# facebook/zstd

Measured on NVIDIA H100. Metric: compress GB/s (input) at level 1, higher is better.
Workload: dtype u8

## Files before the change

### zstd_b200/csrc/zb_api.cu

```cuda
#include <cuda_runtime.h>
#include <stdio.h>
#include <stdlib.h>
#include <string.h>
#include <vector>
#include <mutex>
#include <thread>
#include <new>
#include <time.h>
#include "../../include/zstd_b200.h"
#include "zb_common.h"
#include "zb_kernels.h"

static inline u32 hb32(u32 v) { return 31u - (u32)__builtin_clz(v); }

typedef struct { u32 windowLog, chainLog, hashLog, searchLog, minMatch, targetLength, strategy; } ZbCParams;
struct Row { u8 W, C, H, S, L, TL, strat; };
static const Row kRows[4][5] = {
    { {19,12,13,1,6,1,1}, {19,13,14,1,7,0,1}, {20,15,16,1,6,0,1}, {21,16,17,1,5,0,2}, {21,18,18,1,5,0,2} },
    { {18,12,13,1,5,1,1}, {18,13,14,1,6,0,1}, {18,14,14,1,5,0,2}, {18,16,16,1,4,0,2}, {18,16,16,1,4,0,2} },
    { {17,12,12,1,5,1,1}, {17,12,13,1,6,0,1}, {17,13,15,1,5,0,1}, {17,15,16,2,5,0,2}, {17,17,17,2,4,0,2} },
    { {14,12,13,1,5,1,1}, {14,14,15,1,5,0,1}, {14,14,15,1,4,0,1}, {14,14,15,2,4,0,2}, {14,14,15,2,4,0,2} },
};

static ZbCParams zb_getCParams(int level, u64 srcSize, size_t dictSize)
// ... 55 lines not shown
#define ZB_IMAGE_BYTES (ZB_IMAGE_WORDS * 4u)
#define ZB_MAX_IMAGES 4

#include <atomic>
static std::atomic<int> g_device(-1);

#define ZB_WAVE_SLOTS_MAX 14u
#define ZB_WAVE_SLOTS_DEFAULT 4u
#define ZB_HOST_WAVE_SLOTS_DEFAULT 8u
#define ZB_HOST_WAVE_BLOCKS 384u
struct ZSTD_CDict_s {
    int level;
    const u8* content;
    size_t size;
    size_t contentOff, tail;
    ZbDictEntropy entropy;
    std::mutex* lock;
    int device;
    bool resident;
    u8* d_dict; ZbDictEntropy* d_de; u8* d_image; ZbChunk* d_dictChunk;
    u32 nbImages; ZbParams imagePrm[ZB_MAX_IMAGES];
};

struct ZbPlan;
static void zb_freePlan(struct ZbPlan* p);
struct ZSTD_CCtx_s {
    int device;
    int bindDevice;
    cudaStream_t stream;
    size_t capBlocks, capFrames, capWaves;
    size_t capHeavyBytes[9];
    size_t capChunks; ZbChunk* d_chunks;
    ZbSegMeta* d_segmeta;
    u32 devWaveBlocks;
    cudaStream_t waveStream[ZB_WAVE_SLOTS_MAX + 1];
    u32 waveSlots;
    u32 hostWaveSlots;
    u32 hostWaveBlocks;
    ZbBlock* d_blocks; ZbFrame* d_frames; ZbBlockMeta* d_meta;
    u64* d_seqs; u8* d_lits; u8* d_body; u16* d_dist;
    u16* d_dist2;
    u32* d_far; u32* d_far2;
    u64* d_outOffsets; u64* d_frameSizes; u64* d_totals;
    u8* d_in; size_t d_inCap; u8* d_out; size_t d_outCap;
    ZSTD_CDict* callDict;
    u64* h_totals;
    cudaEvent_t evStart, evK0, evMid, evK1, evK2, evK3, evKEnd, evEnd;
    cudaEvent_t* evWave;
    u32 capEvWaves; bool evWaveTimed;
    ZSTDB200_stats stats;
    int advLevel, advChecksum, advNoDictID;
    ZSTD_CDict* advLocalDict;
    const ZSTD_CDict* advRefCDict;
    struct ZbPlan* plan;
    u8* stIn; size_t stInSize, stInCap;
    u8* stOut; size_t stOutSize, stOutPos, stOutCap;
    int stFrames;
    int advDelims;
    u8* d_seqIn; size_t d_seqInCap;
    void* d_seqTile; size_t d_seqTileCap; void* d_seqBlk; size_t d_seqBlkCap; u64* d_seqCtrl;
};

static double zb_now(void) { struct timespec ts; clock_gettime(CLOCK_MONOTONIC, &ts); return (double)ts.tv_sec + 1e-9 * (double)ts.tv_nsec; }

extern "C" int ZSTDB200_setDevice(int device) { g_device.store(device); return 0; }
int zb_contextDevice(void)
// ... 32 lines not shown
static size_t zb_ctxInit(ZSTD_CCtx* c)
{
    if (c->device >= 0) { CK(cudaSetDevice(c->device)); return 0; }
    int n = 0;
    if (cudaGetDeviceCount(&n) != cudaSuccess || n == 0) { cudaGetLastError(); return ZB_ERR(ZB_error_GENERIC); }
    int dev = c->bindDevice;
    if (dev < 0) { if (cudaGetDevice(&dev) != cudaSuccess) dev = 0; }
    CK(cudaSetDevice(dev));
    cudaStream_t st = nullptr; cudaEvent_t ev[8] = { nullptr, nullptr, nullptr, nullptr, nullptr, nullptr, nullptr, nullptr };
    cudaError_t e = cudaStreamCreateWithFlags(&st, cudaStreamNonBlocking);
    for (int i = 0; i < 8 && e == cudaSuccess; i++) e = cudaEventCreate(&ev[i]);
    if (e == cudaSuccess) {
        static ZbdFseCTable defaults[3]; static std::once_flag once;
        std::call_once(once, [] { zb_buildDefaultTables(defaults); });
        e = zb_upload_default_tables(defaults, st);
        if (e == cudaSuccess) e = cudaStreamSynchronize(st);
    }
    if (e != cudaSuccess) {
        for (int i = 0; i < 8; i++) if (ev[i]) cudaEventDestroy(ev[i]);
        if (st) cudaStreamDestroy(st);
        cudaGetLastError();
        return ZB_ERR(e == cudaErrorMemoryAllocation ? ZB_error_memory_allocation : ZB_error_GENERIC);
    }
    c->stream = st;
    c->evStart = ev[0]; c->evK0 = ev[1]; c->evK1 = ev[2]; c->evK2 = ev[3]; c->evK3 = ev[4]; c->evMid = ev[5]; c->evKEnd = ev[6]; c->evEnd = ev[7];
    c->device = dev;
    return 0;
}

static void zb_freeWorkspace(ZSTD_CCtx* c)
{
    cudaFree(c->d_blocks); cudaFree(c->d_frames); cudaFree(c->d_meta); cudaFree(c->d_seqs); cudaFree(c->d_lits);
    cudaFree(c->d_body); cudaFree(c->d_dist); cudaFree(c->d_dist2); c->d_dist2 = NULL; cudaFree(c->d_segmeta); c->d_segmeta = NULL;
    cudaFree(c->d_far); cudaFree(c->d_far2); c->d_far = NULL; c->d_far2 = NULL; cudaFree(c->d_chunks); c->d_chunks = NULL; c->capChunks = 0; cudaFree(c->d_outOffsets); cudaFree(c->d_frameSizes); cudaFree(c->d_totals);
    cudaFreeHost(c->h_totals);
    c->d_blocks = NULL; c->d_frames = NULL; c->d_meta = NULL; c->d_seqs = NULL; c->d_lits = NULL;
    c->d_body = NULL; c->d_dist = NULL; c->d_outOffsets = NULL; c->d_frameSizes = NULL; c->d_totals = NULL; c->h_totals = NULL;
    c->capBlocks = 0; c->capFrames = 0; c->capWaves = 0; memset(c->capHeavyBytes, 0, sizeof(c->capHeavyBytes));
}

static void zb_freeWaveEvents(ZSTD_CCtx* c)
{
    for (u32 i = 0; i < 4u * c->capEvWaves; i++) if (c->evWave[i]) cudaEventDestroy(c->evWave[i]);
    free(c->evWave); c->evWave = NULL; c->capEvWaves = 0;
}
static size_t zb_ensureWaveEvents(ZSTD_CCtx* c, u32 nbWaves, bool timed)
{
    if (nbWaves <= c->capEvWaves && timed == c->evWaveTimed) return 0;
    zb_freeWaveEvents(c);
    c->evWave = (cudaEvent_t*)calloc(4u * nbWaves, sizeof(cudaEvent_t));
    if (!c->evWave) return ZB_ERR(ZB_error_memory_allocation);
    c->capEvWaves = nbWaves; c->evWaveTimed = timed;
    for (u32 i = 0; i < 4u * nbWaves; i++) {
        cudaError_t const e = cudaEventCreateWithFlags(&c->evWave[i], timed ? cudaEventDefault : cudaEventDisableTiming);
        if (e != cudaSuccess) { zb_freeWaveEvents(c); CK(e); }
    }
    return 0;
}

extern "C" size_t ZSTD_freeCDict(ZSTD_CDict* cd);
extern "C" size_t ZSTD_freeCCtx(ZSTD_CCtx* c)
{
    if (!c) return 0;
    ZbDeviceGuard guard;
    ZSTD_freeCDict(c->advLocalDict); ZSTD_freeCDict(c->callDict);
    free(c->stIn); free(c->stOut);
    zb_freePlan(c->plan);
    if (c->device >= 0) {
        cudaSetDevice(c->device);
        zb_freeWorkspace(c);
        zb_freeWaveEvents(c);
        cudaFree(c->d_in); cudaFree(c->d_out);
        cudaFree(c->d_seqIn); cudaFree(c->d_seqTile); cudaFree(c->d_seqBlk); cudaFree(c->d_seqCtrl);
        for (u32 s = 0; s <= ZB_WAVE_SLOTS_MAX; s++) if (c->waveStream[s]) cudaStreamDestroy(c->waveStream[s]);
        cudaEventDestroy(c->evStart); cudaEventDestroy(c->evK0); cudaEventDestroy(c->evK1);
        cudaEventDestroy(c->evK2); cudaEventDestroy(c->evK3); cudaEventDestroy(c->evMid);
        cudaEventDestroy(c->evKEnd); cudaEventDestroy(c->evEnd);
        cudaStreamDestroy(c->stream);
    }
    free(c);
    return 0;
}

static size_t zb_ensureDesc(ZSTD_CCtx* c, size_t nbBlocks, size_t nbFrames, size_t nbWaves, size_t nbChunks)
{
    if (nbChunks > c->capChunks) {
        cudaFree(c->d_chunks); c->d_chunks = NULL; c->capChunks = 0;
        CK(cudaMalloc(&c->d_chunks, nbChunks * sizeof(ZbChunk)));
        c->capChunks = nbChunks;
    }
    if (nbBlocks > c->capBlocks) {
        cudaFree(c->d_blocks); cudaFree(c->d_outOffsets); c->d_blocks = NULL; c->d_outOffsets = NULL; c->capBlocks = 0;
        CK(cudaMalloc(&c->d_blocks, nbBlocks * sizeof(ZbBlock)));
        CK(cudaMalloc(&c->d_outOffsets, (nbBlocks + 1) * sizeof(u64)));
        c->capBlocks = nbBlocks;
    }
    if (nbFrames > c->capFrames) {
        cudaFree(c->d_frames); cudaFree(c->d_frameSizes); c->d_frames = NULL; c->d_frameSizes = NULL; c->capFrames = 0;
        CK(cudaMalloc(&c->d_frames, nbFrames * sizeof(ZbFrame)));
        CK(cudaMalloc(&c->d_frameSizes, nbFrames * sizeof(u64)));
        c->capFrames = nbFrames;
    }
    if (nbWaves > c->capWaves) {
        cudaFree(c->d_totals); cudaFreeHost(c->h_totals); c->d_totals = NULL; c->h_totals = NULL; c->capWaves = 0;
        CK(cudaMalloc(&c->d_totals, nbWaves * sizeof(u64)));
        CK(cudaMallocHost(&c->h_totals, nbWaves * sizeof(u64)));
        c->capWaves = nbWaves;
    }
    return 0;
}
static size_t zb_ensureHeavy(ZSTD_CCtx* c, size_t nbSlotBlocks, const ZbStrides& sd, bool needDist2, bool needMatch = true)
{
    size_t const nb = nbSlotBlocks;
    size_t const need[9] = { nb * sizeof(ZbBlockMeta), nb * sd.seq * sizeof(u64), nb * (size_t)sd.lit, nb * (size_t)sd.body,
                             nb * (size_t)sd.dist * sizeof(u16), needDist2 ? nb * (size_t)sd.dist * sizeof(u16) : 0,
                             needMatch ? nb * ((sd.dist + ZB_PARSE_SEG - 1u) / ZB_PARSE_SEG) * sizeof(ZbSegMeta) : 0,
                             needMatch ? nb * (size_t)sd.dist * sizeof(u32) : 0, needDist2 ? nb * (size_t)sd.dist * sizeof(u32) : 0 };
    void** const ptr[9] = { (void**)&c->d_meta, (void**)&c->d_seqs, (void**)&c->d_lits, (void**)&c->d_body, (void**)&c->d_dist, (void**)&c->d_dist2,
// ... 159 lines not shown
    if (cd->entropy.present) CK(cudaMemcpyAsync(cd->d_de, &cd->entropy, sizeof(ZbDictEntropy), cudaMemcpyHostToDevice, stream));
    if (shared) CK(cudaStreamSynchronize(stream));
    cd->resident = true;
    return 0;
}

static size_t zb_buildDictImages(ZSTD_CDict* cd, ZbPlan& P, bool shared, cudaStream_t stream)
{
    if (cd->tail < 8) return 0;
    const u8* const d_dictEnd = cd->d_dict + 32 + cd->tail;
    std::lock_guard<std::mutex> g(*cd->lock);
    bool built = false;
    for (size_t gi = 0; gi < P.groups.size(); gi++) {
        ZbParams const& prm = P.groups[gi].prm;
        u32 slot = ~0u;
        for (u32 i = 0; i < cd->nbImages; i++) if (memcmp(&cd->imagePrm[i], &prm, sizeof(prm)) == 0) slot = i;
        if (slot == ~0u) {
            if (cd->nbImages >= ZB_MAX_IMAGES) continue;
            slot = cd->nbImages;
            ZbChunk ch; memset(&ch, 0, sizeof(ch));
            ch.histLen = (u32)cd->tail; ch.dictLen = (u32)cd->tail; ch.size = 0; ch.blockLog = 17;
            CK(cudaMemcpyAsync(cd->d_dictChunk + slot, &ch, sizeof(ZbChunk), cudaMemcpyHostToDevice, stream));
            u32* const img = (u32*)(cd->d_image + (size_t)slot * ZB_IMAGE_BYTES);
            CK(zb_launch_dict_image(d_dictEnd, cd->d_dictChunk + slot, &prm, img, stream));
            cd->imagePrm[slot] = prm; cd->nbImages++; built = true;
        }
        P.groups[gi].image = (const u32*)(cd->d_image + (size_t)slot * ZB_IMAGE_BYTES);
    }
    if (built && shared) CK(cudaStreamSynchronize(stream));
    return 0;
}

static size_t zb_runBlocks(ZSTD_CCtx* c, const ZbPlan& P, const u8* d_src, const u8* d_dictEnd, const ZbDictEntropy* d_de, u32 b0, u32 b1, u32 c0, u32 c1, size_t slot0,
                           cudaStream_t stream, bool timed, unsigned* launches)
{
    for (int phase = 0; phase < 3; phase++) {
        for (size_t g = 0; g < P.groups.size(); g++) {
            ZbGroup const& G = P.groups[g];
            u32 const lo = G.b0 > b0 ? G.b0 : b0, hi = G.b1 < b1 ? G.b1 : b1;
            u32 const clo = G.c0 > c0 ? G.c0 : c0, chi = G.c1 < c1 ? G.c1 : c1;
            if (lo >= hi) continue;
            size_t const s = slot0 + (lo - b0);
            if (phase == 0) {
                bool const df = G.prm.strategy == 2;
                CK(zb_launch_match(d_src, d_dictEnd, d_dictEnd ? G.image : (const u32*)0, c->d_blocks + lo, hi - lo, c->d_chunks + clo, chi - clo, lo, &G.prm, &P.sd,
                                   c->d_dist + s * P.sd.dist, c->d_far + s * P.sd.dist, df ? c->d_dist2 + s * P.sd.dist : (u16*)0, df ? c->d_far2 + s * P.sd.dist : (u32*)0,
                                   c->d_seqs + s * P.sd.seq, c->d_lits + s * P.sd.lit, c->d_meta + s, c->d_segmeta + s * ((P.sd.dist + ZB_PARSE_SEG - 1u) / ZB_PARSE_SEG),
                                   (timed && P.groups.size() == 1) ? c->evMid : (cudaEvent_t)0, stream));
                *launches += df ? 4 : 3;
            } else if (phase == 1) {
                CK(zb_launch_literals(c->d_blocks + lo, hi - lo, &G.prm, &P.sd, d_de, c->d_lits + s * P.sd.lit, c->d_body + s * P.sd.body, c->d_meta + s, stream));
                *launches += 1;
            } else {
                CK(zb_launch_sequences(d_src, c->d_blocks + lo, hi - lo, &G.prm, &P.sd, d_de, c->d_seqs + s * P.sd.seq, c->d_dist + s * P.sd.dist,
                                       c->d_body + s * P.sd.body, c->d_meta + s, stream));
                *launches += 1;
            }
        }
        if (timed) CK(cudaEventRecord(phase == 0 ? c->evK1 : (phase == 1 ? c->evK2 : c->evK3), stream));
    }
    return 0;
}

static u64 zb_xxh64(const u8* p, size_t len)
{
    u64 const P1 = 0x9E3779B185EBCA87ull, P2 = 0xC2B2AE3D27D4EB4Full, P3 = 0x165667B19E3779F9ull, P4 = 0x85EBCA77C2B2AE63ull, P5 = 0x27D4EB2F165667C5ull;
    auto rotl = [](u64 x, int r) { return (x << r) | (x >> (64 - r)); };
    auto rd64 = [](const u8* q) { u64 v; memcpy(&v, q, 8); return v; };
    auto rd32 = [](const u8* q) { u32 v; memcpy(&v, q, 4); return v; };
    auto round = [&](u64 acc, u64 in) { return rotl(acc + in * P2, 31) * P1; };
    auto merge = [&](u64 acc, u64 v) { return (acc ^ round(0, v)) * P1 + P4; };
    const u8* const end = p + len;
    u64 h;
    if (len >= 32) {
        u64 v1 = P1 + P2, v2 = P2, v3 = 0, v4 = 0 - P1;
        const u8* const limit = end - 32;
        do { v1 = round(v1, rd64(p)); v2 = round(v2, rd64(p + 8)); v3 = round(v3, rd64(p + 16)); v4 = round(v4, rd64(p + 24)); p += 32; } while (p <= limit);
        h = rotl(v1, 1) + rotl(v2, 7) + rotl(v3, 12) + rotl(v4, 18);
        h = merge(h, v1); h = merge(h, v2); h = merge(h, v3); h = merge(h, v4);
    } else h = P5;
    h += (u64)len;
// ... 73 lines not shown
    if (deviceMemory) { d_in = (u8*)src; d_out = dst; }
    else {
        if (inEnd + 16 > c->d_inCap) { cudaFree(c->d_in); c->d_in = NULL; c->d_inCap = 0; CK(cudaMalloc(&c->d_in, inEnd + 16)); c->d_inCap = inEnd + 16; }
        if (outCap + 16 > c->d_outCap) { cudaFree(c->d_out); c->d_out = NULL; c->d_outCap = 0; CK(cudaMalloc(&c->d_out, outCap + 16)); c->d_outCap = outCap + 16; }
        d_in = c->d_in; d_out = c->d_out;
        size_t const e = getStream(ZB_WAVE_SLOTS_MAX, &sD2H); if (zb_isErr(e)) return e;
    }
    std::vector<double> hostDone(nbWaves, 0.0);
    double const hostT0 = zb_now();
    unsigned launches = 0;
    size_t err = 0;
    if (!single) CK(cudaEventRecord(c->evStart, sCopy));
    CK(cudaMemcpyAsync(c->d_blocks, P.blocks.data(), nbBlocks * sizeof(ZbBlock), cudaMemcpyHostToDevice, sCopy));
    CK(cudaMemcpyAsync(c->d_frames, P.frames.data(), nbFrames * sizeof(ZbFrame), cudaMemcpyHostToDevice, sCopy));
    CK(cudaMemcpyAsync(c->d_chunks, P.chunks.data(), P.chunks.size() * sizeof(ZbChunk), cudaMemcpyHostToDevice, sCopy));
    if (single) CK(cudaEventRecord(c->evK0, sCopy));
    if (cd && (nbFrames >= 8 || shared)) { size_t const e = zb_buildDictImages(cd, P, shared, sCopy); if (zb_isErr(e)) return e; }
    cudaStream_t lastStream = sCopy;
    for (u32 w = 0; w < nbWaves && !err; w++) {
        u32 const b0 = wb[w], b1 = wb[w + 1];
        size_t const s0 = (size_t)(w % slots) * maxWaveBlocks;
        if (!deviceMemory) {
            u64 lo = ~0ull, hi = 0;
            for (u32 b = b0; b < b1; b++) { u64 const s = P.blocks[b].srcOff, e = s + P.blocks[b].size; if (s < lo) lo = s; if (e > hi) hi = e; }
            if (hi > lo) CK(cudaMemcpyAsync(d_in + lo, src + lo, hi - lo, cudaMemcpyHostToDevice, sCopy));
        }
        cudaStream_t st = sCopy;
        if (!single) {
            CK(cudaEventRecord(evH2D[w], sCopy));
            {   size_t const e = getStream(w % slots, &st); if (zb_isErr(e)) return e; }
            CK(cudaStreamWaitEvent(st, evH2D[w], 0));
        }
        lastStream = st;
        err = zb_runBlocks(c, P, d_in, d_dictEnd, de ? cd->d_de : NULL, b0, b1, wc[w], wc[w + 1], s0, st, single, &launches);
        if (err) break;
        if (w > 0) CK(cudaStreamWaitEvent(st, evStitch[w - 1], 0));
        CK(zb_launch_stitch(d_in, c->d_blocks + b0, b1 - b0, c->d_frames, c->d_body + s0 * P.sd.body, P.sd.body, c->d_meta + s0,
                            c->d_outOffsets + b0, w > 0 ? c->d_totals + (w - 1) : NULL, c->d_totals + w, d_out, outCap, st));
        launches += 2;
        if (!single) CK(cudaEventRecord(evStitch[w], st));
        if (download || timeline) {
            CK(cudaMemcpyAsync(c->h_totals + w, c->d_totals + w, sizeof(u64), cudaMemcpyDeviceToHost, st));
            CK(cudaEventRecord(evSize[w], st));
        }
    }
    double const hostEnq = zb_now() - hostT0;
    std::vector<u64> xxh;
    if (a.checksum && !err && !deviceMemory) {
        xxh.resize(nbFrames);
        size_t const nt = nbFrames < 8 ? nbFrames : 8;
        if (nt <= 1) xxh[0] = zb_xxh64(src + frameOffsets[0], frameSizes[0]);
        else {
            std::vector<std::thread> th;
            for (size_t t = 0; t < nt; t++) th.emplace_back([&, t] { for (size_t f = t; f < nbFrames; f += nt) xxh[f] = zb_xxh64(src + frameOffsets[f], frameSizes[f]); });
            for (size_t t = 0; t < nt; t++) th[t].join();
        }
    }
    if (a.checksum && !err && deviceMemory) { CK(zb_launch_checksums(d_in, c->d_frames, (u32)nbFrames, c->d_outOffsets, d_out, outCap, lastStream)); launches++; }
    bool const wantSizes = a.cSizes != NULL || (a.checksum && !deviceMemory);
    std::vector<u64> fsz;
    u64 prev = 0, total = 0;
    if (download || timeline) {
        for (u32 w = 0; w < nbWaves && !err; w++) {
            CK(cudaEventSynchronize(evSize[w]));
            hostDone[w] = zb_now() - hostT0;
            total = c->h_totals[w];
            if (download && total <= outCap && total > prev) CK(cudaMemcpyAsync(dst + prev, d_out + prev, total - prev, cudaMemcpyDeviceToHost, sD2H));
// ... 595 lines not shown
```

### zstd_b200/csrc/zb_kernels.h

```cpp
#ifndef ZB_KERNELS_H
#define ZB_KERNELS_H
#include <cuda_runtime.h>
#include "zb_common.h"

#ifdef __cplusplus
extern "C" {
#endif

cudaError_t zb_launch_dict_image(const u8* d_dictEnd, const ZbChunk* d_dictChunk, const ZbParams* prm, u32* d_image, cudaStream_t stream);
cudaError_t zb_launch_match(const u8* d_src, const u8* d_dictEnd, const u32* d_image, const ZbBlock* d_blocks, u32 nbBlocks,
                            const ZbChunk* d_chunks, u32 nbChunks, u32 slotFirstBlock, const ZbParams* prm, const ZbStrides* sd,
                            u16* d_dist, u32* d_far, u16* d_dist2, u32* d_far2, u64* d_seqs, u8* d_lits, ZbBlockMeta* d_meta, ZbSegMeta* d_segmeta,
                            cudaEvent_t evMid, cudaStream_t stream);

cudaError_t zb_launch_seq_partition(const void* d_seqs, u32 n, int expl, u64* d_tileLen, u32* d_tileEnds, u64* d_ctrl, cudaStream_t stream);
cudaError_t zb_launch_seq_place(const void* d_seqs, u32 n, int expl, const u64* d_tileLen, const u32* d_tileEnds,
                                u64 srcSize, u64 window, u64 dictContent, u32 blockMax, u32 nbBlocks,
                                u64* d_blockEnd, u32* d_blockSeq, u32* d_blockFirst, u64* d_blockFirstPos, u64* d_ctrl, cudaStream_t stream);
cudaError_t zb_launch_seq_blocks(const u64* d_blockEnd, const u32* d_blockSeq, u32 nbBlocks, u32 blockMax, u32 dictFlag,
                                 ZbBlock* d_blocks, u32* d_blockFirst, u64* d_blockFirstPos, u64* d_ctrl, cudaStream_t stream);
cudaError_t zb_launch_seq_convert(const u8* d_src, const ZbBlock* d_blocks, u32 nbBlocks, const u32* d_blockFirst, const u64* d_blockFirstPos,
                                  const void* d_seqs, u32 n, const ZbParams* prm, const ZbStrides* sd,
                                  u64* d_seqOut, u8* d_lits, ZbBlockMeta* d_meta, cudaStream_t stream);

void zb_buildDefaultTables(ZbdFseCTable* out3);
cudaError_t zb_upload_default_tables(const ZbdFseCTable* host3, cudaStream_t stream);

size_t zb_loadDictionary(ZbDictEntropy* de, const u8* dict, size_t dictSize);

cudaError_t zb_launch_literals(const ZbBlock* d_blocks, u32 nbBlocks, const ZbParams* prm, const ZbStrides* sd, const ZbDictEntropy* d_de,
                               const u8* d_lits, u8* d_body, ZbBlockMeta* d_meta, cudaStream_t stream);

cudaError_t zb_launch_sequences(const u8* d_src, const ZbBlock* d_blocks, u32 nbBlocks, const ZbParams* prm, const ZbStrides* sd, const ZbDictEntropy* d_de,
                                const u64* d_seqs, u16* d_stateBits, u8* d_body, ZbBlockMeta* d_meta, cudaStream_t stream);

cudaError_t zb_launch_stitch(const u8* d_src, const ZbBlock* d_blocks, u32 nbBlocks, const ZbFrame* d_frames,
                             const u8* d_body, u32 bodyStride, const ZbBlockMeta* d_meta,
                             u64* d_outOffsets, const u64* d_base, u64* d_total,
                             u8* d_dst, u64 dstCapacity, cudaStream_t stream);
cudaError_t zb_launch_checksums(const u8* d_src, const ZbFrame* d_frames, u32 nbFrames, const u64* d_outOffsets, u8* d_dst, u64 dstCapacity, cudaStream_t stream);
cudaError_t zb_launch_frame_sizes(const ZbFrame* d_frames, u32 nbFrames, const u64* d_outOffsets,
                                  u64* d_frameSizes, cudaStream_t stream);

#ifdef __cplusplus
}
#endif
// ... 2 lines not shown
```

### zstd_b200/csrc/zb_match.cu

```cuda
#include "zb_device.cuh"
#include "zb_kernels.h"
#include "zb_merge.cuh"

#ifndef WALK_FAST_BC
#define WALK_FAST_BC 1
#endif

template <bool DICT>
__device__ __forceinline__ u32 zb_count_fwd(const ZbSeg& sg, u32 a, u32 offset, u32 be, u32 lane)
{
    u32 fwd = 0;
    while (true) {
        u32 const pa = a + fwd + 8u * lane;
        u32 m;
        if (pa + 8u <= be) {
            u64 const x = zb_seg_ld64x<DICT>(sg, pa) ^ zb_seg_ld64x<DICT>(sg, pa - offset);
            m = x ? (u32)((__ffsll((long long)x) - 1) >> 3) : 8u;
        } else {
            m = 0;
            while (pa + m < be && zb_seg_byte<DICT>(sg, pa + m) == zb_seg_byte<DICT>(sg, pa + m - offset)) m++;
        }
        u32 const inc = __ballot_sync(ZB_FULL, m != 8u);
        if (inc == 0) { fwd += 256u; continue; }
        int const f = __ffs((int)inc) - 1;
// ... 251 lines not shown
        u32 const step = insStep + ((x0 - li) >> 7);
        u32 const pat = zb_walk_pattern_res<P>(step == insStep ? r0 : zb_walk_residue(xa - shift, step), step);
        bool const output = !buildImage && x0 >= H + shift;
        u32 const qb0 = x0 - shift - H;
        size_t const row = output ? (size_t)(cd.firstBlock - slotFirstBlock + (qb0 >> cd.blockLog)) * sd.dist + (qb0 & blockMask) : 0;
        if (zb_walk_batch<MLS, P, true>(table, xa, cur, pat, N, shift, D, total, xLow, xEnd, fbase, dbase, output, distT + row, farT + row)) li = x0 + ZB_BATCH;
        r0 += stepInc; if (r0 >= insStep) r0 -= insStep;
        x0 += ZB_BATCH;
    };
    while (x0 < xEnd) {
        if (WALK_STEADY && x0 >= xIntLoB && x0 + 4u * ZB_BATCH <= xIntHi) {
            if (D != 0u && li < D + shift) li = D + shift;
            do { steadyBatch(rawA, shA); steadyBatch(rawB, shB); } while (x0 + 4u * ZB_BATCH <= xIntHi);
        }
        doBatch(rawA, shA);
        if (x0 >= xEnd) break;
        doBatch(rawB, shB);
    }
    if (buildImage) { __syncthreads(); for (u32 i = t; i < N; i += THREADS) imageOut[i] = table[i]; }
}

#ifndef PARSE_WARPS
#define PARSE_WARPS 8
#endif
#ifndef PARSE_MIN_CTAS
#define PARSE_MIN_CTAS 6
#endif
__device__ __forceinline__ u32 zb_dist_at(const u16* __restrict__ d16, const u32* __restrict__ far, u32 i)
{
    u32 const d = d16[i];
    return d == ZB_FAR ? far[i] : d;
}

template <bool DICT>
__global__ void __launch_bounds__(32 * PARSE_WARPS, DICT ? (40 / PARSE_WARPS) : PARSE_MIN_CTAS)
zb_parse_kernel(const u8* __restrict__ src, const u8* __restrict__ dictEnd, const ZbBlock* __restrict__ blocks, u32 nbBlocks, ZbParams prm, ZbStrides sd,
                const u16* __restrict__ dist, const u32* __restrict__ far, u64* __restrict__ seqs, ZbBlockMeta* __restrict__ meta, ZbSegMeta* __restrict__ segmeta)
{
    u32 const lane = threadIdx.x & 31u;
    u32 const g = blockIdx.x * PARSE_WARPS + (threadIdx.x >> 5);
    u32 const segs = (sd.dist + ZB_PARSE_SEG - 1u) / ZB_PARSE_SEG;
    u32 const b = g / segs, k = g % segs;
    if (b >= nbBlocks) return;
    ZbBlock const bd = blocks[b];
    u64* const myseq = seqs + (size_t)b * sd.seq + (size_t)k * (ZB_PARSE_SEG / 4u);
    const u16* const mydist = dist + (size_t)b * sd.dist;
    const u32* const myfar = far + (size_t)b * sd.dist;
    const u8* const base = src + bd.srcOff - bd.histLen;
    u32 const bs = bd.histLen, blockEnd = bd.histLen + bd.size;
    ZbSeg sg; sg.hi = base; sg.lo = base; sg.split = 0;
    if (DICT && (bd.flags & ZB_FLAG_DICT)) { sg.lo = dictEnd - bd.dictLen; sg.split = bd.dictLen; }

    if (bd.size < 7u) {
        if (lane == 0 && k == 0) {
            ZbBlockMeta m; m.nbSeq = 0; m.litSize = bd.size; m.litSecSize = 0; m.bodySize = bd.size;
            m.type = ZB_BT_RAW; m.forceRaw = 1; m.rleByte = 0; m.pad = 0;
            meta[b] = m;
        }
        return;
    }
    u32 const ss = bs + k * ZB_PARSE_SEG;
    if (ss >= blockEnd) {
        if (lane == 0) { ZbSegMeta z; z.nbSeq = 0; z.pad[0] = z.pad[1] = z.pad[2] = 0; segmeta[(size_t)b * segs + k] = z; }
        return;
    }
    u32 const se = min(ss + ZB_PARSE_SEG, blockEnd);
    u32 const be = blockEnd;

    u32 ip = ss, anchor = ss, searchStart = ss;
    u32 rep1 = 0, rep2 = 0, nbSeq = 0;
    if ((bd.flags & ZB_FLAG_FIRST) && k == 0u) { rep1 = prm.startRep[0]; rep2 = prm.startRep[1]; }

    while (ip < se && ip + 8u <= be) {
        u32 const step = prm.stepSize + ((ip - searchStart) >> 7);
        u32 const p = ip + (lane >> 1) * step + (lane & 1u);
        bool const act = (p < se) && (p + 8u <= be);
// ... 26 lines not shown
        while (tent) {
            int const winner = __ffs((int)tent) - 1;
            probe = __shfl_sync(ZB_FULL, p, winner);
            wtype = __shfl_sync(ZB_FULL, hit, winner);
            u32 const wd = __shfl_sync(ZB_FULL, d, winner);
            back = __shfl_sync(ZB_FULL, myback, winner);
            u32 more = __shfl_sync(ZB_FULL, mymore, winner);
            offset = (wtype == 3u) ? rep2 : ((wtype == 2u) ? rep1 : wd);
            if (wtype == 1u) {
                u32 const f0 = zb_count_fwd<DICT>(sg, probe, offset, be, lane);
                if (f0 < 4u) { tent &= ~(1u << winner); continue; }
                fwdFrom4 = f0 - 4u;
                more = 1u;
            } else {
                fwdFrom4 = zb_count_fwd<DICT>(sg, probe + 4u, offset, be, lane);
            }
            if (more) back += zb_back_coop<DICT>(sg, probe - back, offset, anchor, lane);
            found = true;
            break;
        }
        if (!found) { ip += 16u * step; continue; }
        u32 const ms = probe - back;
        u32 const mlen = back + 4u + fwdFrom4;
        if (wtype == 3u) { u32 const t = rep2; rep2 = rep1; rep1 = t; }
        else if (wtype == 1u) { rep2 = rep1; rep1 = offset; }
        if (lane == 0) myseq[nbSeq] = zb_pack_raw(offset, mlen, ms - bs);
        nbSeq++;
        ip = ms + mlen; anchor = ip; searchStart = ip;
    }
    if (lane == 0) { ZbSegMeta z; z.nbSeq = nbSeq; z.pad[0] = z.pad[1] = z.pad[2] = 0; segmeta[(size_t)b * segs + k] = z; }
}

template <bool DICT>
__global__ void __launch_bounds__(32 * PARSE_WARPS)
zb_parse_dfast_kernel(const u8* __restrict__ src, const u8* __restrict__ dictEnd, const ZbBlock* __restrict__ blocks, u32 nbBlocks, ZbParams prm, ZbStrides sd,
                      const u16* __restrict__ distLong, const u32* __restrict__ farLong, const u16* __restrict__ distShort, const u32* __restrict__ farShort,
                      u64* __restrict__ seqs, ZbBlockMeta* __restrict__ meta, ZbSegMeta* __restrict__ segmeta)
{
    u32 const lane = threadIdx.x & 31u;
    u32 const g = blockIdx.x * PARSE_WARPS + (threadIdx.x >> 5);
    u32 const segs = (sd.dist + ZB_PARSE_SEG - 1u) / ZB_PARSE_SEG;
    u32 const b = g / segs, k = g % segs;
    if (b >= nbBlocks) return;
    ZbBlock const bd = blocks[b];
    u64* const myseq = seqs + (size_t)b * sd.seq + (size_t)k * (ZB_PARSE_SEG / 4u);
    const u16* const dLp = distLong + (size_t)b * sd.dist;
    const u32* const fLp = farLong + (size_t)b * sd.dist;
    const u16* const dSp = distShort + (size_t)b * sd.dist;
    const u32* const fSp = farShort + (size_t)b * sd.dist;
    const u8* const base = src + bd.srcOff - bd.histLen;
    u32 const bs = bd.histLen, blockEnd = bd.histLen + bd.size;
    ZbSeg sg; sg.hi = base; sg.lo = base; sg.split = 0;
    if (DICT && (bd.flags & ZB_FLAG_DICT)) { sg.lo = dictEnd - bd.dictLen; sg.split = bd.dictLen; }

    if (bd.size < 7u) {
        if (lane == 0 && k == 0) {
            ZbBlockMeta m; m.nbSeq = 0; m.litSize = bd.size; m.litSecSize = 0; m.bodySize = bd.size;
            m.type = ZB_BT_RAW; m.forceRaw = 1; m.rleByte = 0; m.pad = 0;
            meta[b] = m;
        }
        return;
    }
    u32 const ss = bs + k * ZB_PARSE_SEG;
    if (ss >= blockEnd) {
        if (lane == 0) { ZbSegMeta z; z.nbSeq = 0; z.pad[0] = z.pad[1] = z.pad[2] = 0; segmeta[(size_t)b * segs + k] = z; }
        return;
    }
    u32 const se = min(ss + ZB_PARSE_SEG, blockEnd);
    u32 const be = blockEnd;
    u32 ip = ss, anchor = ss, searchStart = ss;
    u32 rep1 = 0, rep2 = 0, nbSeq = 0;
    if ((bd.flags & ZB_FLAG_FIRST) && k == 0u) { rep1 = prm.startRep[0]; rep2 = prm.startRep[1]; }

    while (ip < se && ip + 9u <= be) {
        u32 const step = 1u + ((ip - searchStart) >> 8);
        u32 const p = ip + lane * step;
// ... 24 lines not shown
            if (wtype == 3u) { ms = probe; offset = rep2; mlen = 4u + zb_count_fwd<DICT>(sg, probe + 4u, rep2, be, lane); found = true; break; }
            if (wtype == 2u) { ms = probe + 1u; offset = rep1; mlen = 4u + zb_count_fwd<DICT>(sg, probe + 5u, rep1, be, lane); found = true; break; }
            if (wtype == 1u) {
                u32 const f0 = zb_count_fwd<DICT>(sg, probe, wL, be, lane);
                if (f0 >= 8u) {
                    u32 const back = zb_back_coop<DICT>(sg, probe, wL, anchor, lane);
                    ms = probe - back; offset = wL; mlen = back + f0; found = true; break;
                }
                if (lane == (u32)winner) hit = dS ? 4u : 0u;
                if (wS == 0u) { tent &= ~(1u << winner); }
                continue;
            }
            {   u32 const f0 = zb_count_fwd<DICT>(sg, probe, wS, be, lane);
                if (f0 < 4u) { tent &= ~(1u << winner); if (lane == (u32)winner) hit = 0u; continue; }
                u32 mp = probe, mo = wS, ml = f0;
                if (wL1) {
                    u32 const f1 = zb_count_fwd<DICT>(sg, probe + 1u, wL1, be, lane);
                    if (f1 >= 8u && f1 > ml) { mp = probe + 1u; mo = wL1; ml = f1; }
                }
                u32 const back = zb_back_coop<DICT>(sg, mp, mo, anchor, lane);
                ms = mp - back; offset = mo; mlen = back + ml; wtype = 1u; found = true; break;
            }
        }
        if (!found) { ip += 32u * step; continue; }
        if (wtype == 3u) { u32 const t = rep2; rep2 = rep1; rep1 = t; }
        else if (wtype == 1u) { rep2 = rep1; rep1 = offset; }
        if (lane == 0) myseq[nbSeq] = zb_pack_raw(offset, mlen, ms - bs);
        nbSeq++;
        ip = ms + mlen; anchor = ip; searchStart = ip;
    }
    if (lane == 0) { ZbSegMeta z; z.nbSeq = nbSeq; z.pad[0] = z.pad[1] = z.pad[2] = 0; segmeta[(size_t)b * segs + k] = z; }
}

struct ZbRepHist { u32 r1, r2, r3; };
__device__ __forceinline__ u32 zb_rep_code(ZbRepHist& h, u32 off, u32 ll)
{
    u32 code;
    if (ll > 0u) {
        if (off == h.r1) return 1u;
        if (off == h.r2) { code = 2u; h.r2 = h.r1; h.r1 = off; return code; }
        if (off == h.r3) { code = 3u; h.r3 = h.r2; h.r2 = h.r1; h.r1 = off; return code; }
    } else {
        if (off == h.r2) { code = 1u; h.r2 = h.r1; h.r1 = off; return code; }
        if (off == h.r3) { code = 2u; h.r3 = h.r2; h.r2 = h.r1; h.r1 = off; return code; }
        if (h.r1 > 1u && off == h.r1 - 1u) { code = 3u; h.r3 = h.r2; h.r2 = h.r1; h.r1 = off; return code; }
    }
    h.r3 = h.r2; h.r2 = h.r1; h.r1 = off;
    return off + 3u;
}

#ifndef MERGE_MIN_CTAS
#define MERGE_MIN_CTAS 6
#endif
#define SEG_SLOTS (ZB_PARSE_SEG / 4u)
__global__ void __launch_bounds__(MERGE_THREADS, MERGE_MIN_CTAS)
zb_merge_segments_kernel(const u8* __restrict__ src, const ZbBlock* __restrict__ blocks, ZbParams prm, ZbStrides sd, const ZbSegMeta* __restrict__ segmeta,
                         u64* __restrict__ seqs, u8* __restrict__ lits, ZbBlockMeta* __restrict__ meta)
{
    __shared__ u32 sPos[MERGE_TILE], sLit[MERGE_TILE], sLen[MERGE_TILE], sOff[MERGE_TILE];
    __shared__ u32 wsumL[MERGE_THREADS / 32], wsumA[MERGE_THREADS / 32], wmaxU[MERGE_THREADS / 32], wmaxK[MERGE_THREADS / 32];
    __shared__ u32 sR2[MERGE_TILE], sRep[3];
    __shared__ u32 baseL, baseA, carryEnd;
    __shared__ u32 gFirst[ZB_PARSE_SEGS], gCnt[ZB_PARSE_SEGS], gBase[ZB_PARSE_SEGS], gCur[ZB_PARSE_SEGS], gPm[ZB_PARSE_SEGS], gPl[ZB_PARSE_SEGS];
    __shared__ u32 gTotal;
    u32 const b = blockIdx.x, tid = threadIdx.x, lane = tid & 31u, warp = tid >> 5;
    ZbBlock const bd = blocks[b];
// ... 118 lines not shown
template <int MLS>
static cudaError_t zb_launch_walk_m(const u8* d_src, const u8* d_dictEnd, const ZbChunk* d_chunks, u32 nbChunks, u32 N, u32 insStep, const ZbStrides& sd,
                                    u32 slotFirstBlock, u16* d_dist, u32* d_far, const u32* d_imageIn, u32* d_imageOut, cudaStream_t stream)
{
    size_t const smem = (size_t)N * 4u;
    if (smem <= 56u * 1024u)  return zb_launch_walk_p<MLS, WALK_P_SMALL>(d_src, d_dictEnd, d_chunks, nbChunks, N, insStep, sd, slotFirstBlock, d_dist, d_far, d_imageIn, d_imageOut, stream);
    if (smem <= 113u * 1024u) return zb_launch_walk_p<MLS, WALK_P_MID>(d_src, d_dictEnd, d_chunks, nbChunks, N, insStep, sd, slotFirstBlock, d_dist, d_far, d_imageIn, d_imageOut, stream);
    return zb_launch_walk_p<MLS, 1>(d_src, d_dictEnd, d_chunks, nbChunks, N, insStep, sd, slotFirstBlock, d_dist, d_far, d_imageIn, d_imageOut, stream);
}
static cudaError_t zb_launch_walk(const u8* d_src, const u8* d_dictEnd, const ZbChunk* d_chunks, u32 nbChunks, u32 mls, u32 N, u32 insStep, const ZbStrides& sd,
                                  u32 slotFirstBlock, u16* d_dist, u32* d_far, const u32* d_imageIn, u32* d_imageOut, cudaStream_t stream)
{
    switch (mls) {
    case 4: return zb_launch_walk_m<4>(d_src, d_dictEnd, d_chunks, nbChunks, N, insStep, sd, slotFirstBlock, d_dist, d_far, d_imageIn, d_imageOut, stream);
    case 5: return zb_launch_walk_m<5>(d_src, d_dictEnd, d_chunks, nbChunks, N, insStep, sd, slotFirstBlock, d_dist, d_far, d_imageIn, d_imageOut, stream);
    case 6: return zb_launch_walk_m<6>(d_src, d_dictEnd, d_chunks, nbChunks, N, insStep, sd, slotFirstBlock, d_dist, d_far, d_imageIn, d_imageOut, stream);
    case 7: return zb_launch_walk_m<7>(d_src, d_dictEnd, d_chunks, nbChunks, N, insStep, sd, slotFirstBlock, d_dist, d_far, d_imageIn, d_imageOut, stream);
    default: return zb_launch_walk_m<8>(d_src, d_dictEnd, d_chunks, nbChunks, N, insStep, sd, slotFirstBlock, d_dist, d_far, d_imageIn, d_imageOut, stream);
    }
}

extern "C" cudaError_t zb_launch_dict_image(const u8* d_dictEnd, const ZbChunk* d_dictChunk, const ZbParams* prm, u32* d_image, cudaStream_t stream)
{
    ZbStrides sd; sd.dist = ZB_BLOCK_MAX; sd.seq = ZB_SEQ_STRIDE; sd.lit = ZB_LIT_STRIDE; sd.body = ZB_BODY_STRIDE; sd.state = ZB_STATE_STRIDE;
    cudaError_t e = zb_launch_walk(nullptr, d_dictEnd, d_dictChunk, 1, prm->mls, prm->tableN, prm->insStep, sd, 0, nullptr, nullptr, nullptr, d_image, stream);
    if (e == cudaSuccess && prm->strategy == 2)
        e = zb_launch_walk(nullptr, d_dictEnd, d_dictChunk, 1, 8, prm->tableNLong, prm->insStep, sd, 0, nullptr, nullptr, nullptr, d_image + prm->tableN, stream);
    return e;
}

extern "C" cudaError_t zb_launch_match(const u8* d_src, const u8* d_dictEnd, const u32* d_image, const ZbBlock* d_blocks, u32 nbBlocks,
                                       const ZbChunk* d_chunks, u32 nbChunks, u32 slotFirstBlock, const ZbParams* prm, const ZbStrides* sdp,
                                       u16* d_dist, u32* d_far, u16* d_dist2, u32* d_far2, u64* d_seqs, u8* d_lits, ZbBlockMeta* d_meta, ZbSegMeta* d_segmeta,
                                       cudaEvent_t evMid, cudaStream_t stream)
{
    if (nbBlocks == 0) return cudaSuccess;
    ZbStrides const sd = *sdp;
    cudaError_t e;
    u32 const segs = (sd.dist + ZB_PARSE_SEG - 1u) / ZB_PARSE_SEG;
    u32 const sgrid = (u32)(((u64)nbBlocks * segs + PARSE_WARPS - 1) / PARSE_WARPS);
    if (prm->strategy == 2) {
        e = zb_launch_walk(d_src, d_dictEnd, d_chunks, nbChunks, 8, prm->tableNLong, prm->insStep, sd, slotFirstBlock, d_dist, d_far, d_image ? d_image + prm->tableN : nullptr, nullptr, stream); if (e != cudaSuccess) return e;
        e = zb_launch_walk(d_src, d_dictEnd, d_chunks, nbChunks, prm->mls, prm->tableN, prm->insStep, sd, slotFirstBlock, d_dist2, d_far2, d_image, nullptr, stream); if (e != cudaSuccess) return e;
        if (evMid) cudaEventRecord(evMid, stream);
        if (d_dictEnd) zb_parse_dfast_kernel<true><<<sgrid, 32 * PARSE_WARPS, 0, stream>>>(d_src, d_dictEnd, d_blocks, nbBlocks, *prm, sd, d_dist, d_far, d_dist2, d_far2, d_seqs, d_meta, d_segmeta);
        else           zb_parse_dfast_kernel<false><<<sgrid, 32 * PARSE_WARPS, 0, stream>>>(d_src, nullptr, d_blocks, nbBlocks, *prm, sd, d_dist, d_far, d_dist2, d_far2, d_seqs, d_meta, d_segmeta);
    } else {
        e = zb_launch_walk(d_src, d_dictEnd, d_chunks, nbChunks, prm->mls, prm->tableN, prm->insStep, sd, slotFirstBlock, d_dist, d_far, d_image, nullptr, stream); if (e != cudaSuccess) return e;
        if (evMid) cudaEventRecord(evMid, stream);
        if (d_dictEnd) zb_parse_kernel<true><<<sgrid, 32 * PARSE_WARPS, 0, stream>>>(d_src, d_dictEnd, d_blocks, nbBlocks, *prm, sd, d_dist, d_far, d_seqs, d_meta, d_segmeta);
        else           zb_parse_kernel<false><<<sgrid, 32 * PARSE_WARPS, 0, stream>>>(d_src, nullptr, d_blocks, nbBlocks, *prm, sd, d_dist, d_far, d_seqs, d_meta, d_segmeta);
    }
    if (segs == 1u && sd.dist <= 8192u)
        zb_merge_small_kernel<<<(nbBlocks + MERGE_THREADS / 32u - 1u) / (MERGE_THREADS / 32u), MERGE_THREADS, 0, stream>>>(d_src, d_blocks, nbBlocks, *prm, sd, d_segmeta, d_seqs, d_lits, d_meta);
    else
        zb_merge_segments_kernel<<<nbBlocks, MERGE_THREADS, 0, stream>>>(d_src, d_blocks, *prm, sd, d_segmeta, d_seqs, d_lits, d_meta);
    return cudaGetLastError();
}
```

Baseline: 93.82.

## Make parse kernels persistent with atomic work-stealing over segments

Turns the parse and dfast-parse kernels into persistent kernels. The grid is capped at the resident CTA count, and each warp fetches segment indices from a global atomic counter per wave slot, which is reset with a memset before each launch. The goal is to balance uneven per-segment parse work and cut tail imbalance. In exchange it adds a memset launch, occupancy queries on every launch, and one atomic per segment. Segment order no longer follows block order.

```diff
diff --git a/zstd_b200/csrc/zb_api.cu b/zstd_b200/csrc/zb_api.cu
--- a/zstd_b200/csrc/zb_api.cu
+++ b/zstd_b200/csrc/zb_api.cu
@@ -111,6 +111,7 @@
     size_t capHeavyBytes[9];
     size_t capChunks; ZbChunk* d_chunks;
     ZbSegMeta* d_segmeta;
+    u32* d_parseCtr;
     u32 devWaveBlocks;
     cudaStream_t waveStream[ZB_WAVE_SLOTS_MAX + 1];
     u32 waveSlots;
@@ -209,7 +210,7 @@
 {
     cudaFree(c->d_blocks); cudaFree(c->d_frames); cudaFree(c->d_meta); cudaFree(c->d_seqs); cudaFree(c->d_lits);
     cudaFree(c->d_body); cudaFree(c->d_dist); cudaFree(c->d_dist2); c->d_dist2 = NULL; cudaFree(c->d_segmeta); c->d_segmeta = NULL;
-    cudaFree(c->d_far); cudaFree(c->d_far2); c->d_far = NULL; c->d_far2 = NULL; cudaFree(c->d_chunks); c->d_chunks = NULL; c->capChunks = 0; cudaFree(c->d_outOffsets); cudaFree(c->d_frameSizes); cudaFree(c->d_totals);
+    cudaFree(c->d_far); cudaFree(c->d_far2); c->d_far = NULL; c->d_far2 = NULL; cudaFree(c->d_chunks); c->d_chunks = NULL; c->capChunks = 0; cudaFree(c->d_parseCtr); c->d_parseCtr = NULL; cudaFree(c->d_outOffsets); cudaFree(c->d_frameSizes); cudaFree(c->d_totals);
     cudaFreeHost(c->h_totals);
     c->d_blocks = NULL; c->d_frames = NULL; c->d_meta = NULL; c->d_seqs = NULL; c->d_lits = NULL;
     c->d_body = NULL; c->d_dist = NULL; c->d_outOffsets = NULL; c->d_frameSizes = NULL; c->d_totals = NULL; c->h_totals = NULL;
@@ -261,6 +262,7 @@
 
 static size_t zb_ensureDesc(ZSTD_CCtx* c, size_t nbBlocks, size_t nbFrames, size_t nbWaves, size_t nbChunks)
 {
+    if (!c->d_parseCtr) CK(cudaMalloc(&c->d_parseCtr, ZB_WAVE_SLOTS_MAX * sizeof(u32)));
     if (nbChunks > c->capChunks) {
         cudaFree(c->d_chunks); c->d_chunks = NULL; c->capChunks = 0;
         CK(cudaMalloc(&c->d_chunks, nbChunks * sizeof(ZbChunk)));
@@ -486,7 +488,7 @@
 }
 
 static size_t zb_runBlocks(ZSTD_CCtx* c, const ZbPlan& P, const u8* d_src, const u8* d_dictEnd, const ZbDictEntropy* d_de, u32 b0, u32 b1, u32 c0, u32 c1, size_t slot0,
-                           cudaStream_t stream, bool timed, unsigned* launches)
+                           u32* d_parseCtr, cudaStream_t stream, bool timed, unsigned* launches)
 {
     for (int phase = 0; phase < 3; phase++) {
         for (size_t g = 0; g < P.groups.size(); g++) {
@@ -500,7 +502,7 @@
                 CK(zb_launch_match(d_src, d_dictEnd, d_dictEnd ? G.image : (const u32*)0, c->d_blocks + lo, hi - lo, c->d_chunks + clo, chi - clo, lo, &G.prm, &P.sd,
                                    c->d_dist + s * P.sd.dist, c->d_far + s * P.sd.dist, df ? c->d_dist2 + s * P.sd.dist : (u16*)0, df ? c->d_far2 + s * P.sd.dist : (u32*)0,
                                    c->d_seqs + s * P.sd.seq, c->d_lits + s * P.sd.lit, c->d_meta + s, c->d_segmeta + s * ((P.sd.dist + ZB_PARSE_SEG - 1u) / ZB_PARSE_SEG),
-                                   (timed && P.groups.size() == 1) ? c->evMid : (cudaEvent_t)0, stream));
+                                   d_parseCtr, (timed && P.groups.size() == 1) ? c->evMid : (cudaEvent_t)0, stream));
                 *launches += df ? 4 : 3;
             } else if (phase == 1) {
                 CK(zb_launch_literals(c->d_blocks + lo, hi - lo, &G.prm, &P.sd, d_de, c->d_lits + s * P.sd.lit, c->d_body + s * P.sd.body, c->d_meta + s, stream));
@@ -640,7 +642,7 @@
             CK(cudaStreamWaitEvent(st, evH2D[w], 0));
         }
         lastStream = st;
-        err = zb_runBlocks(c, P, d_in, d_dictEnd, de ? cd->d_de : NULL, b0, b1, wc[w], wc[w + 1], s0, st, single, &launches);
+        err = zb_runBlocks(c, P, d_in, d_dictEnd, de ? cd->d_de : NULL, b0, b1, wc[w], wc[w + 1], s0, c->d_parseCtr + w % slots, st, single, &launches);
         if (err) break;
         if (w > 0) CK(cudaStreamWaitEvent(st, evStitch[w - 1], 0));
         CK(zb_launch_stitch(d_in, c->d_blocks + b0, b1 - b0, c->d_frames, c->d_body + s0 * P.sd.body, P.sd.body, c->d_meta + s0,
diff --git a/zstd_b200/csrc/zb_kernels.h b/zstd_b200/csrc/zb_kernels.h
--- a/zstd_b200/csrc/zb_kernels.h
+++ b/zstd_b200/csrc/zb_kernels.h
@@ -11,7 +11,7 @@
 cudaError_t zb_launch_match(const u8* d_src, const u8* d_dictEnd, const u32* d_image, const ZbBlock* d_blocks, u32 nbBlocks,
                             const ZbChunk* d_chunks, u32 nbChunks, u32 slotFirstBlock, const ZbParams* prm, const ZbStrides* sd,
                             u16* d_dist, u32* d_far, u16* d_dist2, u32* d_far2, u64* d_seqs, u8* d_lits, ZbBlockMeta* d_meta, ZbSegMeta* d_segmeta,
-                            cudaEvent_t evMid, cudaStream_t stream);
+                            u32* d_parseCtr, cudaEvent_t evMid, cudaStream_t stream);
 
 cudaError_t zb_launch_seq_partition(const void* d_seqs, u32 n, int expl, u64* d_tileLen, u32* d_tileEnds, u64* d_ctrl, cudaStream_t stream);
 cudaError_t zb_launch_seq_place(const void* d_seqs, u32 n, int expl, const u64* d_tileLen, const u32* d_tileEnds,
diff --git a/zstd_b200/csrc/zb_match.cu b/zstd_b200/csrc/zb_match.cu
--- a/zstd_b200/csrc/zb_match.cu
+++ b/zstd_b200/csrc/zb_match.cu
@@ -307,16 +307,19 @@
     return d == ZB_FAR ? far[i] : d;
 }
 
+__device__ __forceinline__ u32 zb_parse_next(u32* __restrict__ ctr, u32 lane)
+{
+    u32 g = 0;
+    if (lane == 0) g = atomicAdd(ctr, 1u);
+    return __shfl_sync(ZB_FULL, g, 0);
+}
+
 template <bool DICT>
-__global__ void __launch_bounds__(32 * PARSE_WARPS, DICT ? (40 / PARSE_WARPS) : PARSE_MIN_CTAS)
-zb_parse_kernel(const u8* __restrict__ src, const u8* __restrict__ dictEnd, const ZbBlock* __restrict__ blocks, u32 nbBlocks, ZbParams prm, ZbStrides sd,
-                const u16* __restrict__ dist, const u32* __restrict__ far, u64* __restrict__ seqs, ZbBlockMeta* __restrict__ meta, ZbSegMeta* __restrict__ segmeta)
-{
-    u32 const lane = threadIdx.x & 31u;
-    u32 const g = blockIdx.x * PARSE_WARPS + (threadIdx.x >> 5);
-    u32 const segs = (sd.dist + ZB_PARSE_SEG - 1u) / ZB_PARSE_SEG;
+__device__ __forceinline__ void zb_parse_segment(u32 g, u32 lane, const u8* __restrict__ src, const u8* __restrict__ dictEnd, const ZbBlock* __restrict__ blocks,
+                                                 const ZbParams& prm, const ZbStrides& sd, u32 segs,
+                                                 const u16* __restrict__ dist, const u32* __restrict__ far, u64* __restrict__ seqs, ZbBlockMeta* __restrict__ meta, ZbSegMeta* __restrict__ segmeta)
+{
     u32 const b = g / segs, k = g % segs;
-    if (b >= nbBlocks) return;
     ZbBlock const bd = blocks[b];
     u64* const myseq = seqs + (size_t)b * sd.seq + (size_t)k * (ZB_PARSE_SEG / 4u);
     const u16* const mydist = dist + (size_t)b * sd.dist;
@@ -409,16 +412,24 @@
 }
 
 template <bool DICT>
-__global__ void __launch_bounds__(32 * PARSE_WARPS)
-zb_parse_dfast_kernel(const u8* __restrict__ src, const u8* __restrict__ dictEnd, const ZbBlock* __restrict__ blocks, u32 nbBlocks, ZbParams prm, ZbStrides sd,
-                      const u16* __restrict__ distLong, const u32* __restrict__ farLong, const u16* __restrict__ distShort, const u32* __restrict__ farShort,
-                      u64* __restrict__ seqs, ZbBlockMeta* __restrict__ meta, ZbSegMeta* __restrict__ segmeta)
+__global__ void __launch_bounds__(32 * PARSE_WARPS, DICT ? (40 / PARSE_WARPS) : PARSE_MIN_CTAS)
+zb_parse_kernel(const u8* __restrict__ src, const u8* __restrict__ dictEnd, const ZbBlock* __restrict__ blocks, u32 nbBlocks, ZbParams prm, ZbStrides sd,
+                const u16* __restrict__ dist, const u32* __restrict__ far, u64* __restrict__ seqs, ZbBlockMeta* __restrict__ meta, ZbSegMeta* __restrict__ segmeta,
+                u32* __restrict__ ctr)
 {
     u32 const lane = threadIdx.x & 31u;
-    u32 const g = blockIdx.x * PARSE_WARPS + (threadIdx.x >> 5);
     u32 const segs = (sd.dist + ZB_PARSE_SEG - 1u) / ZB_PARSE_SEG;
+    for (u32 g; (g = zb_parse_next(ctr, lane)) < nbBlocks * segs; )
+        zb_parse_segment<DICT>(g, lane, src, dictEnd, blocks, prm, sd, segs, dist, far, seqs, meta, segmeta);
+}
+
+template <bool DICT>
+__device__ __forceinline__ void zb_parse_dfast_segment(u32 g, u32 lane, const u8* __restrict__ src, const u8* __restrict__ dictEnd, const ZbBlock* __restrict__ blocks,
+                                                       const ZbParams& prm, const ZbStrides& sd, u32 segs,
+                                                       const u16* __restrict__ distLong, const u32* __restrict__ farLong, const u16* __restrict__ distShort, const u32* __restrict__ farShort,
+                                                       u64* __restrict__ seqs, ZbBlockMeta* __restrict__ meta, ZbSegMeta* __restrict__ segmeta)
+{
     u32 const b = g / segs, k = g % segs;
-    if (b >= nbBlocks) return;
     ZbBlock const bd = blocks[b];
     u64* const myseq = seqs + (size_t)b * sd.seq + (size_t)k * (ZB_PARSE_SEG / 4u);
     const u16* const dLp = distLong + (size_t)b * sd.dist;
@@ -509,6 +520,18 @@
     if (lane == 0) { ZbSegMeta z; z.nbSeq = nbSeq; z.pad[0] = z.pad[1] = z.pad[2] = 0; segmeta[(size_t)b * segs + k] = z; }
 }
 
+template <bool DICT>
+__global__ void __launch_bounds__(32 * PARSE_WARPS)
+zb_parse_dfast_kernel(const u8* __restrict__ src, const u8* __restrict__ dictEnd, const ZbBlock* __restrict__ blocks, u32 nbBlocks, ZbParams prm, ZbStrides sd,
+                      const u16* __restrict__ distLong, const u32* __restrict__ farLong, const u16* __restrict__ distShort, const u32* __restrict__ farShort,
+                      u64* __restrict__ seqs, ZbBlockMeta* __restrict__ meta, ZbSegMeta* __restrict__ segmeta, u32* __restrict__ ctr)
+{
+    u32 const lane = threadIdx.x & 31u;
+    u32 const segs = (sd.dist + ZB_PARSE_SEG - 1u) / ZB_PARSE_SEG;
+    for (u32 g; (g = zb_parse_next(ctr, lane)) < nbBlocks * segs; )
+        zb_parse_dfast_segment<DICT>(g, lane, src, dictEnd, blocks, prm, sd, segs, distLong, farLong, distShort, farShort, seqs, meta, segmeta);
+}
+
 struct ZbRepHist { u32 r1, r2, r3; };
 __device__ __forceinline__ u32 zb_rep_code(ZbRepHist& h, u32 off, u32 ll)
 {
@@ -693,24 +716,37 @@
 extern "C" cudaError_t zb_launch_match(const u8* d_src, const u8* d_dictEnd, const u32* d_image, const ZbBlock* d_blocks, u32 nbBlocks,
                                        const ZbChunk* d_chunks, u32 nbChunks, u32 slotFirstBlock, const ZbParams* prm, const ZbStrides* sdp,
                                        u16* d_dist, u32* d_far, u16* d_dist2, u32* d_far2, u64* d_seqs, u8* d_lits, ZbBlockMeta* d_meta, ZbSegMeta* d_segmeta,
-                                       cudaEvent_t evMid, cudaStream_t stream)
+                                       u32* d_parseCtr, cudaEvent_t evMid, cudaStream_t stream)
 {
     if (nbBlocks == 0) return cudaSuccess;
     ZbStrides const sd = *sdp;
     cudaError_t e;
     u32 const segs = (sd.dist + ZB_PARSE_SEG - 1u) / ZB_PARSE_SEG;
-    u32 const sgrid = (u32)(((u64)nbBlocks * segs + PARSE_WARPS - 1) / PARSE_WARPS);
+    u32 const ctas = (u32)(((u64)nbBlocks * segs + PARSE_WARPS - 1) / PARSE_WARPS);
+    auto grid = [&](const void* kernel, u32* g) -> cudaError_t {
+        int dev = 0, sms = 0, per = 0;
+        cudaError_t r = cudaGetDevice(&dev);
+        if (r == cudaSuccess) r = cudaDeviceGetAttribute(&sms, cudaDevAttrMultiProcessorCount, dev);
+        if (r == cudaSuccess) r = cudaOccupancyMaxActiveBlocksPerMultiprocessor(&per, kernel, 32 * PARSE_WARPS, 0);
+        if (r != cudaSuccess) return r;
+        u32 const resident = (u32)(sms * (per > 0 ? per : 1));
+        *g = ctas < resident ? ctas : resident;
+        return cudaMemsetAsync(d_parseCtr, 0, sizeof(u32), stream);
+    };
+    u32 sgrid = 0;
     if (prm->strategy == 2) {
         e = zb_launch_walk(d_src, d_dictEnd, d_chunks, nbChunks, 8, prm->tableNLong, prm->insStep, sd, slotFirstBlock, d_dist, d_far, d_image ? d_image + prm->tableN : nullptr, nullptr, stream); if (e != cudaSuccess) return e;
         e = zb_launch_walk(d_src, d_dictEnd, d_chunks, nbChunks, prm->mls, prm->tableN, prm->insStep, sd, slotFirstBlock, d_dist2, d_far2, d_image, nullptr, stream); if (e != cudaSuccess) return e;
         if (evMid) cudaEventRecord(evMid, stream);
-        if (d_dictEnd) zb_parse_dfast_kernel<true><<<sgrid, 32 * PARSE_WARPS, 0, stream>>>(d_src, d_dictEnd, d_blocks, nbBlocks, *prm, sd, d_dist, d_far, d_dist2, d_far2, d_seqs, d_meta, d_segmeta);
-        else           zb_parse_dfast_kernel<false><<<sgrid, 32 * PARSE_WARPS, 0, stream>>>(d_src, nullptr, d_blocks, nbBlocks, *prm, sd, d_dist, d_far, d_dist2, d_far2, d_seqs, d_meta, d_segmeta);
+        e = grid(d_dictEnd ? (const void*)zb_parse_dfast_kernel<true> : (const void*)zb_parse_dfast_kernel<false>, &sgrid); if (e != cudaSuccess) return e;
+        if (d_dictEnd) zb_parse_dfast_kernel<true><<<sgrid, 32 * PARSE_WARPS, 0, stream>>>(d_src, d_dictEnd, d_blocks, nbBlocks, *prm, sd, d_dist, d_far, d_dist2, d_far2, d_seqs, d_meta, d_segmeta, d_parseCtr);
+        else           zb_parse_dfast_kernel<false><<<sgrid, 32 * PARSE_WARPS, 0, stream>>>(d_src, nullptr, d_blocks, nbBlocks, *prm, sd, d_dist, d_far, d_dist2, d_far2, d_seqs, d_meta, d_segmeta, d_parseCtr);
     } else {
         e = zb_launch_walk(d_src, d_dictEnd, d_chunks, nbChunks, prm->mls, prm->tableN, prm->insStep, sd, slotFirstBlock, d_dist, d_far, d_image, nullptr, stream); if (e != cudaSuccess) return e;
         if (evMid) cudaEventRecord(evMid, stream);
-        if (d_dictEnd) zb_parse_kernel<true><<<sgrid, 32 * PARSE_WARPS, 0, stream>>>(d_src, d_dictEnd, d_blocks, nbBlocks, *prm, sd, d_dist, d_far, d_seqs, d_meta, d_segmeta);
-        else           zb_parse_kernel<false><<<sgrid, 32 * PARSE_WARPS, 0, stream>>>(d_src, nullptr, d_blocks, nbBlocks, *prm, sd, d_dist, d_far, d_seqs, d_meta, d_segmeta);
+        e = grid(d_dictEnd ? (const void*)zb_parse_kernel<true> : (const void*)zb_parse_kernel<false>, &sgrid); if (e != cudaSuccess) return e;
+        if (d_dictEnd) zb_parse_kernel<true><<<sgrid, 32 * PARSE_WARPS, 0, stream>>>(d_src, d_dictEnd, d_blocks, nbBlocks, *prm, sd, d_dist, d_far, d_seqs, d_meta, d_segmeta, d_parseCtr);
+        else           zb_parse_kernel<false><<<sgrid, 32 * PARSE_WARPS, 0, stream>>>(d_src, nullptr, d_blocks, nbBlocks, *prm, sd, d_dist, d_far, d_seqs, d_meta, d_segmeta, d_parseCtr);
     }
     if (segs == 1u && sd.dist <= 8192u)
         zb_merge_small_kernel<<<(nbBlocks + MERGE_THREADS / 32u - 1u) / (MERGE_THREADS / 32u), MERGE_THREADS, 0, stream>>>(d_src, d_blocks, nbBlocks, *prm, sd, d_segmeta, d_seqs, d_lits, d_meta);
```

Result: faster. 94.85, median of 6 (+1.1%).
